# retinal-information-processing-lab/gaussian_processes

Measured on AMD Instinct MI355X. Metric: GP fits/sec (kernel+chol+solve+grad loglik) at N=8192 d=256, higher is better.
Workload: dtype f64; 1 GPU; N=8192 d=256 single cell f64, one M-step closure evaluation with 6 gradients (BASELINE configs[2], headline); N=8192, d=256, parallelism=independent units over 1 GPU(s), one process per GPU, no data-path collective

## Files before the change

gaussian_processes_amd/_lib.py:

```python
from __future__ import annotations

import ctypes
import os

from .build import lib_path

vp, i32, i64, f64 = ctypes.c_void_p, ctypes.c_int, ctypes.c_int64, ctypes.c_double
pd = ctypes.POINTER(ctypes.c_double)



class DevGemmArgs(ctypes.Structure):
    _fields_ = ([(n, vp) for n in ("A", "B", "C")] + [(n, i64) for n in ("lda", "ldb", "ldc", "sA", "sB", "sC")] +
                [("alpha", f64), ("beta", f64)] +
                [(n, vp) for n in ("sk_ws", "aux", "sumsq", "Ap", "Bp", "Cp", "auxp", "sumsqp")] +
                [(n, ctypes.c_int32) for n in ("M", "N", "K", "a_kmajor", "b_kmajor", "out_lower", "a_tri", "b_tri", "batch",
                                               "split_k", "tile", "walk", "epi", "nptr", "k_slabs")])


class DevGemmRoute(ctypes.Structure):
    _fields_ = [(n, ctypes.c_int32) for n in ("rc", "tile", "sk_first", "xcd", "stages", "half_occ", "edge", "epi",
                                              "sumsq_entries", "blocks", "pair", "slabs")]


_SIGS = {
    "gpfit_version": (i32, []),
    "gpfit_last_error": (ctypes.c_char_p, []),
    "gpfit_dgemm": (i32, [vp, i32, i32, i32, i32, i32, f64, vp, i64, vp, i64, f64, vp, i64, i32, i32, i32]),
    "gpfit_dgemm_ex": (i32, [vp, i32, i32, i32, i32, i32, f64, vp, i64, vp, i64, f64, vp, i64, i32, i32, i32, i32, i32]),
    "gpfit_ctx_create": (i32, [i32, i64, i64, i64, ctypes.POINTER(vp)]),
    "gpfit_ctx_destroy": (None, [vp]),
    "gpfit_check_limits": (i32, [pd, pd, pd]),
    "gpfit_localker_mask": (i32, [pd, i32, i32, vp, ctypes.POINTER(i64)]),
    "gpfit_localker": (i32, [vp, vp, pd, i32, i32, vp, i64, vp, vp]),
    "gpfit_acosker": (i32, [vp, vp, f64, vp, i64, i64, vp, i64, i64, i64, vp, i64, vp, vp, i64, vp]),
    "gpfit_acosker_pullback": (i32, [vp, vp, f64, vp, i64, i64, vp, i64, i64, i64, vp, i64, vp, i64, vp, vp, i64, pd]),
    "gpfit_acosker_diag": (i32, [vp, vp, f64, vp, i64, i64, i64, vp, i64, vp, vp, vp]),
    "gpfit_fit_eval": (i32, [vp, vp, pd, pd, pd, i32, i32, vp, i64, i64, vp, vp, vp, i64, f64, f64, i32, pd,
                             vp, vp, vp]),
    "gpfit_potrf": (i32, [vp, vp, vp, i64, i64, vp, i64, vp, i64, pd, ctypes.POINTER(i32)]),
    "gpfit_potrf_append": (i32, [vp, vp, vp, i64, vp, i64, i64, vp, pd, ctypes.POINTER(i32)]),
    "gpfit_potrf_append_block": (i32, [vp, vp, vp, i64, vp, i64, i64, i64, vp, i64, pd, ctypes.POINTER(i32)]),
    "gpfit_estep": (i32, [vp, vp, vp, i64, i64, vp, vp, vp, f64, vp, vp, i64]),
    "gpfit_estep_projected": (i32, [vp, vp, vp, i64, vp, i64, vp, i64, i64, i64, vp, vp, vp, f64, vp, vp, i64, vp, vp,
                                    vp]),
    "gpfit_estep_projected_damped": (i32, [vp, vp, vp, i64, vp, i64, vp, i64, vp, i64, vp, i64, i64, i64, vp, vp, vp, f64, f64,
                                           vp, vp, i64, ctypes.POINTER(i32)]),
    "gpfit_fparam_eval": (i32, [vp, vp, vp, vp, vp, i64, f64, i32, f64, vp, pd]),
    "gpfit_fparam_lbfgs": (i32, [vp, vp, vp, vp, vp, i64, f64, i32, f64, i32, i32, f64, f64, f64, vp, pd]),
    "gpfit_estep_chain": (i32, [vp, vp, vp, i64, vp, i64, vp, i64, i64, i64, vp, vp, vp, vp, vp, i64, vp, vp, f64, i32, f64,
                                i32, i32, i32, f64, f64, f64, pd]),
    "gpfit_estep_chain_full": (i32, [vp, vp, vp, i64, i64, vp, vp, vp, vp, vp, i64, vp, vp, f64, i32, f64, i32, i32, i32, f64,
                                     f64, f64, pd]),
    "gpfit_estep_chain_batch": (i32, [vp, i32, vp, vp, vp, vp, vp, vp, vp, i64, vp, vp, vp, vp, vp, vp, vp, vp, vp, pd, i32, pd,
                                      i32, i32, i32, f64, f64, f64, pd]),
# ... 8 lines not shown
    "gpfit_elbo_batch": (i32, [vp, i32, vp, vp, vp, vp, vp, vp, vp, vp, vp, ctypes.POINTER(i32), pd, vp, vp, vp, i64, pd, pd, pd,
                               ctypes.POINTER(i32)]),
    "gpfit_subspace_sweeps": (i32, [vp, vp, vp, i64, i64, i64, vp, vp, vp, vp, i32, pd, i32, ctypes.POINTER(i32)]),
    "gpfit_subspace_sweeps_batch": (i32, [vp, i32, vp, vp, i64, i64, i64, vp, vp, vp, vp, ctypes.POINTER(i32), vp, i32,
                                          ctypes.POINTER(i32)]),
    "gpfit_fparam_lbfgs_host": (i32, [vp, vp, vp, i64, f64, i32, f64, i32, i32, f64, f64, f64, vp, pd]),
    "gpfit_set_profile": (i32, [vp, i32]),
    "gpfit_get_profile": (i32, [vp, pd]),
    "gpfit_get_phases": (i32, [vp, pd]),
    "gpfit_last_enqueue_ms": (f64, [vp]),
    "gpfit_fit_eval_f32": (i32, [vp, vp, pd, pd, pd, i32, i32, vp, i64, i64, vp, vp, vp, i64, f64, f64, i32, pd,
                                 vp, vp, vp]),
    "gpfit_fit_eval_finish": (i32, [vp, pd]),
    "gpfit_fit_eval_batch": (i32, [vp, i32, vp, pd, pd, pd, i32, i32, vp, i64, i64, vp, vp, vp, i64, pd, pd, i32, pd,
                                   ctypes.POINTER(i32)]),
    "gpfit_fit_eval_batch_f32": (i32, [vp, i32, vp, pd, pd, pd, i32, i32, vp, i64, i64, vp, vp, vp, i64, pd, pd, i32, pd,
                                       ctypes.POINTER(i32)]),
    "gpfit_fit_eval_projected": (i32, [vp, vp, pd, pd, pd, i32, i32, vp, i64, i64, vp, vp, i64, i64, vp, vp, i64, f64, f64, pd]),
    "gpfit_fit_eval_projected_batch": (i32, [vp, i32, vp, pd, pd, pd, i32, i32, vp, i64, i64, vp, vp, vp, vp, vp, vp, vp, pd, pd,
                                             pd, ctypes.POINTER(i32)]),
    "gpfit_fit_eval_sparse": (i32, [vp, vp, pd, pd, pd, i32, i32, vp, i64, i64, vp, i64, i64, vp, vp, i64, i64, vp, vp, i64,
                                    f64, f64, pd]),
    "gpfit_fit_eval_sparse_batch": (i32, [vp, i32, vp, pd, pd, pd, i32, i32, vp, i64, i64, vp, i64, i64, vp, vp, vp, vp, vp,
                                          vp, vp, pd, pd, pd, ctypes.POINTER(i32)]),
    "gpfit_grad_pullback": (i32, [vp, vp, pd, i32, i32, vp, i64, i64, vp, i64, vp, pd]),
    "gpfit_nd_utility": (i32, [vp, vp, vp, i64, vp, i32, vp]),
    "gpfit_probe_mfma_f64": (i32, [vp, vp, i32, i32]),
    "gpfit_probe_stream_copy": (i32, [vp, vp, vp, i64]),
    "gpfit_dev_gemm_route": (i32, [i32, ctypes.POINTER(DevGemmArgs), ctypes.POINTER(DevGemmArgs), ctypes.POINTER(DevGemmRoute)]),
    "gpfit_dev_gemm_plan": (i64, [i32, ctypes.POINTER(DevGemmArgs), i32, ctypes.POINTER(ctypes.c_int32), i64]),
    "gpfit_dev_gemm": (i32, [vp, i32, ctypes.POINTER(DevGemmArgs), ctypes.POINTER(DevGemmArgs)]),
    "gpfit_dev_ctx_copy": (i32, [vp, ctypes.c_char_p, i64, vp, i64, i32]),
    "gpfit_dev_ctx_fill": (i32, [vp, ctypes.c_char_p, i32]),
}

_lib = None


class GpfitError(RuntimeError):
    pass


def exported_symbols():
    return sorted(_SIGS)


def load():
    global _lib
    if _lib is not None:
        return _lib
    path = lib_path()
    if not os.path.exists(path):
        raise GpfitError(
            f"{path} not found: build it with `python -m gaussian_processes_amd.build` "
            "(there is no CPU fallback for the GP fit path)")
    lib = ctypes.CDLL(path)
    for name, (res, args) in _SIGS.items():
        fn = getattr(lib, name)
        fn.restype = res
        fn.argtypes = args
    _lib = lib
    return lib


def last_error() -> str:
    return load().gpfit_last_error().decode(errors="replace")
# ... 11 lines not shown
```

gaussian_processes_amd/csrc/api_dev.hip:

```cpp
#include "gemm_core.h"
#include "context.h"
#include "gpfit_mi355x.h"

#include <cstring>

namespace gpfit {
namespace {

template <typename R>
int fill(const gpfit_dev_gemm_args& d, GemmArgsT<R>& g) {
  g = GemmArgsT<R>{};
  g.A = (const R*)d.A; g.B = (const R*)d.B; g.C = (R*)d.C;
  g.lda = d.lda; g.ldb = d.ldb; g.ldc = d.ldc;
  g.M = d.M; g.N = d.N; g.K = d.K;
  g.alpha = d.alpha; g.beta = d.beta;
  g.a_kmajor = d.a_kmajor; g.b_kmajor = d.b_kmajor;
  g.out_lower = d.out_lower; g.a_tri = d.a_tri; g.b_tri = d.b_tri;
  g.batch = d.batch > 0 ? d.batch : 1;
  g.sA = d.sA; g.sB = d.sB; g.sC = d.sC;
  g.split_k = d.split_k > 0 ? d.split_k : 1;
  g.k_slabs = d.k_slabs > 0 ? d.k_slabs : 0;
  g.tile = d.tile;
  g.reverse = d.walk & 15;
  g.half_occ = (d.walk >> 4) & 1;
  g.sk_ws = d.sk_ws;
  g.epi = d.epi;
  g.aux = (R*)d.aux;
  g.sumsq = d.sumsq;
  g.nptr = d.nptr;
  if (d.nptr < 0 || d.nptr > GEMM_MAXB) return d.nptr < 0 ? -3 : 0;
  for (int b = 0; b < d.nptr; ++b) {
    if (!d.Ap || !d.Bp || !d.Cp) return -3;
    g.Ap[b] = (const R*)d.Ap[b];
// ... 62 lines not shown
      w[3] = std::min(kr.end, (z + 1) * sp.ks * SLAB_TILE);
    }
    return need;
  }
  if (kind != 2) return -3;
  if (r.sched != GEMM_STREAMK) return -1;
  const int first = r.sk_first;
  SkHostPlan p;
  if (streamk_plan_host(a, first, p) != 0) return -1;
  const int64_t nt = (int64_t)p.tiles.size(), nfix = (int64_t)p.fix_tile.size(), nslot = (int64_t)p.fix_slot.size();
  const int64_t need = 8 + 5 * nt + nfix + (nfix + 1) + nslot;
  if (need > cap || !out) return need;
  out[0] = first; out[1] = (int32_t)nt; out[2] = p.total; out[3] = p.blocks; out[4] = p.per_block;
  out[5] = (int32_t)nfix; out[6] = (int32_t)nslot;
  out[7] = (int32_t)(SK_WS_BYTES / ((size_t)TILE * TILE * sizeof(double)));
  int32_t* w = out + 8;
  for (const SkTile& t : p.tiles) { *w++ = t.row0; *w++ = t.col0; *w++ = t.kbeg; *w++ = t.ksteps; *w++ = t.prefix; }
  std::memcpy(w, p.fix_tile.data(), nfix * sizeof(int)); w += nfix;
  std::memcpy(w, p.fix_ptr.data(), (nfix + 1) * sizeof(int)); w += nfix + 1;
  std::memcpy(w, p.fix_slot.data(), nslot * sizeof(int));
  return need;
}

template <typename R>
int run(hipStream_t s, const gpfit_dev_gemm_args& d, const gpfit_dev_gemm_args* d2) {
  GemmArgsT<R> a, b;
  if (fill(d, a) != 0 || (d2 && fill(*d2, b) != 0)) {
    set_error("gpfit_dev_gemm: a pointer batch needs its pointer arrays");
    return -3;
  }
  return d2 ? launch_gemm_pair(a, b, gemm_pair_shape(a, b), s) : launch_gemm(a, s);
}

struct CtxBuf { void* p; int64_t bytes; };
CtxBuf ctx_buffer(gpfit_ctx* c, const char* name) {
  const int64_t np = c->np_cap, dp = c->dp_cap, nn = np * np * 8;
  const struct { const char* n; double* p; int64_t bytes; } tab[] = {
      {"Abuf", c->Abuf, nn}, {"Tbuf", c->Tbuf, nn}, {"Wbuf", c->Wbuf, nn}, {"Zbuf", c->Zbuf, nn}, {"Cos", c->Cos, nn},
      {"TmpV", c->TmpV, nn}, {"Xm", c->Xm, np * dp * 8}, {"Xt2", c->Xt2, np * dp * 8}, {"Ybuf", c->Ybuf, np * dp * 8},
      {"Mmat", c->Mmat, dp * dp * 8}, {"Cmat", c->Cmat, dp * dp * 8}, {"tvec", c->tvec, 2 * np * 8}, {"bv", c->bv, np * 8},
      {"q", c->q, np * 8}, {"wl", c->wl, np * 8}, {"q2", c->q2, np * 8}, {"dq1", c->dq1, np * 8}, {"dq2", c->dq2, np * 8}};
  for (const auto& t : tab)
    if (std::strcmp(t.n, name) == 0) return {t.p, t.bytes};
  return {nullptr, 0};
}

}
}

extern "C" {

int gpfit_dev_gemm_route(int is_f32, const gpfit_dev_gemm_args* args, const gpfit_dev_gemm_args* pair_args,
                         gpfit_dev_gemm_route_t* out) {
  if (!args || !out) return -3;
  return is_f32 ? gpfit::route<float>(*args, pair_args, *out) : gpfit::route<double>(*args, pair_args, *out);
}

int64_t gpfit_dev_gemm_plan(int is_f32, const gpfit_dev_gemm_args* args, int kind, int32_t* out, int64_t cap) {
  if (!args) return -3;
  return is_f32 ? gpfit::plan<float>(*args, kind, out, cap) : gpfit::plan<double>(*args, kind, out, cap);
}

int gpfit_dev_gemm(void* stream, int is_f32, const gpfit_dev_gemm_args* args, const gpfit_dev_gemm_args* pair_args) {
  if (!args) return -3;
  return is_f32 ? gpfit::run<float>((hipStream_t)stream, *args, pair_args)
                : gpfit::run<double>((hipStream_t)stream, *args, pair_args);
}

int gpfit_dev_ctx_copy(gpfit_ctx* ctx, const char* name, int64_t offset, void* dev, int64_t bytes, int to_ctx) {
  if (!ctx || !name || !dev || offset < 0 || bytes < 0 || ctx->pend.active) return -3;
  gpfit::DeviceGuard guard(ctx->device);
  const gpfit::CtxBuf b = gpfit::ctx_buffer(ctx, name);
  if (!b.p || offset + bytes > b.bytes) return -3;
  GP_HIP(hipDeviceSynchronize());
  char* w = (char*)b.p + offset;
  GP_HIP(hipMemcpy(to_ctx ? (void*)w : dev, to_ctx ? dev : (void*)w, (size_t)bytes, hipMemcpyDeviceToDevice));
  GP_HIP(hipDeviceSynchronize());
  return 0;
}

int gpfit_dev_ctx_fill(gpfit_ctx* ctx, const char* name, int byte) {
  if (!ctx || !name || ctx->pend.active) return -3;
  gpfit::DeviceGuard guard(ctx->device);
  const gpfit::CtxBuf b = gpfit::ctx_buffer(ctx, name);
  if (!b.p) return -3;
  GP_HIP(hipDeviceSynchronize());
  GP_HIP(hipMemset(b.p, byte, (size_t)b.bytes));
  GP_HIP(hipDeviceSynchronize());
  return 0;
}

}
```

gaussian_processes_amd/csrc/common.h:

```cpp
#pragma once
#include <hip/hip_runtime.h>
#include <stdint.h>
#include <stdio.h>
#include <string>

namespace gpfit {

constexpr double PI32 = 3.1415927410125732;

constexpr int TILE = 128;
constexpr int TRMV_ROWS = 128;
constexpr int KTILE = 16;

void set_error(const std::string& msg);

#define GP_HIP(expr)                                                                     \
  do {                                                                                   \
    hipError_t _e = (expr);                                                              \
    if (_e != hipSuccess) {                                                              \
      gpfit::set_error(std::string(#expr) + ": " + hipGetErrorString(_e));               \
      return -100;                                                                       \
    }                                                                                    \
  } while (0)

#define GP_TRY(expr)            \
  do {                          \
    int _rc = (expr);           \
    if (_rc != 0) return _rc;   \
  } while (0)

inline int64_t round_up(int64_t x, int64_t m) { return (x + m - 1) / m * m; }

constexpr int GEMM_MAXB = 32;

template <typename R>
struct GemmArgsT {
  const R* A;
  const R* B;
  R* C;
  int64_t lda, ldb, ldc;
  int M, N, K;
// ... 114 lines not shown
```

gaussian_processes_amd/csrc/elementwise.hip:

```cpp
#include "kernels.h"

#include <algorithm>

namespace gpfit {

__device__ __forceinline__ double wave_sum(double v) {
#pragma unroll
  for (int o = 32; o > 0; o >>= 1) v += __shfl_down(v, o);
  return v;
}

__device__ __forceinline__ double block_sum(double v, double* sh) {
  const int lane = threadIdx.x & 63, wave = threadIdx.x >> 6;
  const int nw = (blockDim.x + 63) >> 6;
  v = wave_sum(v);
  __syncthreads();
  if (lane == 0) sh[wave] = v;
  __syncthreads();
  if (wave == 0) {
    double t = (lane < nw) ? sh[lane] : 0.0;
    t = wave_sum(t);
    if (lane == 0) sh[16] = t;
  }
  __syncthreads();
  return sh[16];
}

__device__ __forceinline__ double lin_pm1(int i, int n) {
  if (n <= 1) return -1.0;
  const double step = 2.0 / (double)(n - 1);
  return (i < n / 2) ? fma(step, (double)i, -1.0) : fma(-step, (double)(n - 1 - i), 1.0);
}

// ... 611 lines not shown
}
__global__ void dot_group_kernel(PerUnit<double*> x, PerUnit<double*> y, int n, PerUnit<double*> out) {
  __shared__ double sh[17];
  const int u = blockIdx.y;
  dot_body<double>(x[u], y[u], n, out[u], sh);
}
int launch_dot_group(int n_units, PerUnit<double*> x, PerUnit<double*> y, int n, PerUnit<double*> out, hipStream_t s) {
  hipLaunchKernelGGL(dot_group_kernel, dim3(1, n_units), dim3(1024), 0, s, x, y, n, out);
  GP_HIP(hipGetLastError());
  return 0;
}

template <typename R>
int launch_dot(const R* x, const R* y, int n, double* out, hipStream_t s) {
  hipLaunchKernelGGL(dot_kernel<R>, dim3(1), dim3(1024), 0, s, x, y, n, out);
  GP_HIP(hipGetLastError());
  return 0;
}

template <typename R>
__global__ __launch_bounds__(256) void moments_kernel(const R* __restrict__ Kvec, const R* __restrict__ q,
                                                      const R* __restrict__ Cos, int64_t ldc, const R* __restrict__ V,
                                                      int64_t ldv, const R* __restrict__ m, const R* __restrict__ r, int n,
                                                      double A, double lambda0, R* __restrict__ lam_m,
                                                      R* __restrict__ lam_var, R* __restrict__ f, R* __restrict__ wl,
                                                      double* __restrict__ scal, double* __restrict__ part,
                                                      int* __restrict__ ticket) {
  __shared__ double sh[17];
  __shared__ bool last;
  double s_rm = 0.0, s_r = 0.0, s_f = 0.0;
  const int i = blockIdx.x * 256 + threadIdx.x;
  if (i < n) {
    const double c = (double)Cos[(int64_t)i * ldc + i];
    const double delta = acos(c);
    const double J = (sqrt(1.0 - c * c) + PI32 * c - delta * c) / PI32;
    const double qi = (double)q[i];
    const double kii = qi * qi * J;
    const double lv = (double)Kvec[i] - kii + (double)V[(int64_t)i * ldv + i];
    const double lm = (double)m[i];
    const double fi = exp(A * lm + 0.5 * A * A * lv + lambda0);
    const double g = 1.0 - J - (PI32 - delta) * (1.0 - c) / PI32;
    lam_m[i] = (R)lm;
    lam_var[i] = (R)lv;
    f[i] = (R)fi;
    wl[i] = (R)(-0.5 * A * A * fi * g);
    s_rm = (double)r[i] * lm;
    s_r = (double)r[i];
    s_f = fi;
  }
  s_rm = block_sum(s_rm, sh);
  s_r = block_sum(s_r, sh);
  s_f = block_sum(s_f, sh);
  if (threadIdx.x == 0) {
    part[blockIdx.x * 3 + 0] = s_rm;
    part[blockIdx.x * 3 + 1] = s_r;
    part[blockIdx.x * 3 + 2] = s_f;
    __threadfence();
    last = (atomicAdd(ticket, 1) == (int)gridDim.x - 1);
  }
  __syncthreads();
  if (!last) return;
  __threadfence();
  if (threadIdx.x < 3) {
    double v = 0.0;
    for (int b = 0; b < (int)gridDim.x; ++b)
      v += __hip_atomic_load(&part[b * 3 + threadIdx.x], __ATOMIC_RELAXED, __HIP_MEMORY_SCOPE_AGENT);
    scal[threadIdx.x] = v;
  }
  if (threadIdx.x == 0) *ticket = 0;
}

template <typename R>
int launch_moments(const R* Kvec, const R* q, const R* Cos, int64_t ldc, const R* V, int64_t ldv, const R* m,
                   const R* r, int n, double A, double lambda0, R* lam_m, R* lam_var, R* f, R* wl, double* scal,
                   double* part, int* ticket, hipStream_t s) {
  hipLaunchKernelGGL(moments_kernel<R>, dim3((n + 255) / 256), dim3(256), 0, s, Kvec, q, Cos, ldc, V, ldv, m, r, n, A,
                     lambda0, lam_m, lam_var, f, wl, scal, part, ticket);
  GP_HIP(hipGetLastError());
  return 0;
}

template <typename R>
__global__ __launch_bounds__(256) void adjoint_kernel(const R* __restrict__ W, const R* __restrict__ Cos, int64_t ld,
                                                      const R* __restrict__ b, const R* __restrict__ q, int n,
                                                      int np, R* __restrict__ Aout, double* __restrict__ upart,
                                                      double* __restrict__ vpart, double* __restrict__ sumA_part) {
  __shared__ double colsum[4][64];
  __shared__ double sh[17];
  int ti, tj;
  {
    const int t = blockIdx.x;
    int i = (int)((sqrt(8.0 * (double)t + 1.0) - 1.0) * 0.5);
    while ((i + 1) * (i + 2) / 2 <= t) ++i;
    while (i * (i + 1) / 2 > t) --i;
    ti = i;
    tj = t - i * (i + 1) / 2;
  }
  const bool diag = (ti == tj);
  const int tx = threadIdx.x & 63, ty = threadIdx.x >> 6;
  const int j = tj * 64 + tx;
  const double qj = (double)q[j], bj = (double)b[j];
  double csum = 0.0, asum = 0.0;
  for (int rr = ty; rr < 64; rr += 4) {
    const int i = ti * 64 + rr;
    double aw = 0.0, bm = 0.0;
    if (i < n && j < n) {
      const int64_t o = (diag && i < j) ? ((int64_t)j * ld + i) : ((int64_t)i * ld + j);
      const double w = (double)W[o] - 0.5 * (double)b[i] * bj;
      const double c = (double)Cos[o];
      aw = w * (PI32 - acos(c)) / PI32;
      bm = w * sqrt(1.0 - c * c) / PI32;
    }
    Aout[(int64_t)i * ld + j] = (R)((diag && i <= j) ? (i == j ? 0.5 * aw : 0.0) : aw);
    asum += aw;
    const double rs = wave_sum(bm * qj);
    if (tx == 0) upart[(int64_t)tj * np + i] = rs;
    csum += bm * (double)q[i];
  }
  colsum[ty][tx] = csum;
  __syncthreads();
  if (!diag && ty == 0) vpart[(int64_t)ti * np + j] = colsum[0][tx] + colsum[1][tx] + colsum[2][tx] + colsum[3][tx];
  asum = block_sum(asum, sh);
  if (threadIdx.x == 0) sumA_part[blockIdx.x] = diag ? asum : 2.0 * asum;
}

template <typename R>
__global__ __launch_bounds__(256) void adjoint_u_kernel(const double* __restrict__ upart, const double* __restrict__ vpart,
                                                        int nt64, const R* __restrict__ q, const R* __restrict__ wl, int n,
                                                        int np, R* __restrict__ tvec, double* __restrict__ uq) {
  __shared__ double sl[8][33];
  const int li = threadIdx.x & 31, z = threadIdx.x >> 5;
  const int i = blockIdx.x * 32 + li;
  double u = 0.0;
  if (i < n) {
    const int T = i >> 6;
#pragma unroll 4
    for (int t = z; t < nt64; t += 8) u += (t <= T ? upart : vpart)[(int64_t)t * np + i];
  }
  sl[z][li] = u;
  __syncthreads();
  if (z != 0 || i >= np) return;
  if (i >= n) {
    tvec[i] = (R)0;
    uq[i] = 0.0;
    return;
  }
  u = sl[0][li];
#pragma unroll
  for (int k = 1; k < 8; ++k) u += sl[k][li];
  const double v = u / (double)q[i];
  uq[i] = v;
  tvec[i] = (R)(v - (double)wl[i]);
}

template <typename R>
__global__ void adjoint_sums_kernel(const double* __restrict__ uq, const R* __restrict__ wl, int n,
                                    const double* __restrict__ sumA_part, int ntile_tri, double* __restrict__ out) {
  __shared__ double sh[17];
  const int b = blockIdx.x;
  double v = 0.0;
  if (b == 0) for (int i = threadIdx.x; i < n; i += blockDim.x) v += uq[i];
  else if (b == 1) for (int i = threadIdx.x; i < n; i += blockDim.x) v += (double)wl[i];
  else for (int i = threadIdx.x; i < ntile_tri; i += blockDim.x) v += sumA_part[i];
  v = block_sum(v, sh);
  if (threadIdx.x == 0) out[b] = v;
}

__global__ __launch_bounds__(256) void adjoint_rect_kernel(const double* __restrict__ W, int64_t ldw,
                                                           const double* __restrict__ Cos, int64_t ldc,
                                                           const double* __restrict__ q1,
                                                           const double* __restrict__ q2, int n1, int n2, int np1,
                                                           int np2, double* __restrict__ Aout, int64_t lda,
                                                           double* __restrict__ upart, double* __restrict__ vpart,
                                                           double* __restrict__ tile_sum) {
  __shared__ double colsum[4][64];
  __shared__ double sh[17];
  const int tj = blockIdx.x, ti = blockIdx.y;
  const int tx = threadIdx.x & 63, ty = threadIdx.x >> 6;
  const int j = tj * 64 + tx;
  const double qj = (j < n2) ? q2[j] : 0.0;
  double csum = 0.0, asum = 0.0;
  for (int rr = ty; rr < 64; rr += 4) {
    const int i = ti * 64 + rr;
    double aw = 0.0, bm = 0.0;
    if (i < n1 && j < n2) {
      const double w = W[(int64_t)i * ldw + j];
      const double c = Cos[(int64_t)i * ldc + j];
      aw = w * (PI32 - acos(c)) / PI32;
      bm = w * sqrt(1.0 - c * c) / PI32;
    }
    Aout[(int64_t)i * lda + j] = aw;
    asum += aw;
    const double rs = wave_sum(bm * qj);
    if (tx == 0) upart[(int64_t)tj * np1 + i] = rs;
    csum += (i < n1) ? bm * q1[i] : 0.0;
  }
  colsum[ty][tx] = csum;
  __syncthreads();
  if (ty == 0) vpart[(int64_t)ti * np2 + j] = colsum[0][tx] + colsum[1][tx] + colsum[2][tx] + colsum[3][tx];
  asum = block_sum(asum, sh);
  if (threadIdx.x == 0) tile_sum[ti * gridDim.x + tj] = asum;
}

__global__ __launch_bounds__(256) void adjoint_rect_reduce_kernel(const double* __restrict__ part, int nt,
                                                                  const double* __restrict__ q,
                                                                  const double* __restrict__ extra, int n, int np,
                                                                  double* __restrict__ tvec, double* __restrict__ uq) {
  __shared__ double sl[8][33];
  const int li = threadIdx.x & 31, z = threadIdx.x >> 5;
  const int i = blockIdx.x * 32 + li;
  double u = 0.0;
  if (i < n) {
#pragma unroll 4
    for (int t = z; t < nt; t += 8) u += part[(int64_t)t * np + i];
  }
  sl[z][li] = u;
  __syncthreads();
  if (z != 0 || i >= np) return;
  if (i >= n) {
    tvec[i] = 0.0;
    uq[i] = 0.0;
    return;
  }
  u = sl[0][li];
#pragma unroll
  for (int k = 1; k < 8; ++k) u += sl[k][li];
  const double v = u / q[i];
  uq[i] = v;
// ... 168 lines not shown
  if (i >= n || j >= i) return;
  const double a = A[(int64_t)i * lda + j], b = A[(int64_t)j * lda + i];
  const double v = (a + b) / 2.0;
  A[(int64_t)i * lda + j] = v;
  A[(int64_t)j * lda + i] = v;
}
__global__ void symmetrize_avg_kernel(double* __restrict__ A, int64_t lda, int n) { symmetrize_avg_body(A, lda, n); }
__global__ void symmetrize_avg_group_kernel(PerUnit<double*> A, int64_t lda, PerUnit<int> n) {
  const int u = blockIdx.z;
  symmetrize_avg_body(A[u], lda, n[u]);
}
int launch_symmetrize_avg_group(int n_units, PerUnit<double*> A, int64_t lda, PerUnit<int> n, hipStream_t s) {
  int nmax = 0;
  for (int u = 0; u < n_units; ++u) nmax = std::max(nmax, n.v[u]);
  if (nmax <= 0) return 0;
  hipLaunchKernelGGL(symmetrize_avg_group_kernel, dim3((nmax + 255) / 256, nmax, n_units), dim3(256), 0, s, A, lda, n);
  GP_HIP(hipGetLastError());
  return 0;
}

int launch_symmetrize_avg(double* A, int64_t lda, int n, hipStream_t s) {
  hipLaunchKernelGGL(symmetrize_avg_kernel, dim3((n + 255) / 256, n), dim3(256), 0, s, A, lda, n);
  GP_HIP(hipGetLastError());
  return 0;
}

__global__ void dk_sigma0_kernel(const double* __restrict__ Cos, int64_t ldc, const double* __restrict__ q1,
                                 const double* __restrict__ q2, int n1, int n2, double s0,
                                 double* __restrict__ dK, int64_t ldk) {
  const int j = blockIdx.x * blockDim.x + threadIdx.x, i = blockIdx.y;
  if (i >= n1 || j >= n2) return;
  const double c = Cos[(int64_t)i * ldc + j];
  const double a = q1[i], b = q2[j], qq = a * b;
  const double delta = acos(c);
  const double J = (sqrt(1.0 - c * c) + PI32 * c - delta * c) / PI32;
  const double dqq = s0 * s0 * (b / a + a / b);
  const double dcos = (2.0 * s0 * s0 - c * dqq) / qq;
  const double dJ = -(delta - PI32) * dcos / PI32;
  dK[(int64_t)i * ldk + j] = (qq * dJ + dqq * J) / s0;
}

int launch_dk_sigma0(const double* Cos, int64_t ldc, const double* q1, const double* q2, int n1, int n2,
                     double s0, double* dK, int64_t ldk, hipStream_t s) {
  hipLaunchKernelGGL(dk_sigma0_kernel, dim3((n2 + 255) / 256, n1), dim3(256), 0, s, Cos, ldc, q1, q2, n1, n2, s0,
                     dK, ldk);
  GP_HIP(hipGetLastError());
  return 0;
}

__global__ void dq_kernel(const double* __restrict__ Xt, const double* __restrict__ XDt, int64_t ld, int dp,
                          int n, const double* __restrict__ q, double* __restrict__ dq, double* __restrict__ h) {
  const int i = blockIdx.x * blockDim.x + threadIdx.x;
  if (i >= n) return;
  double v = 0.0;
  for (int k = 0; k < dp; ++k) v += Xt[(int64_t)k * ld + i] * XDt[(int64_t)k * ld + i];
  if (h) h[i] = v;
  if (dq) dq[i] = 0.5 * v / q[i];
}

int launch_dq(const double* Xt, const double* XDt, int64_t ld, int dp, int n, const double* q, double* dq,
              double* h, hipStream_t s) {
  hipLaunchKernelGGL(dq_kernel, dim3((n + 255) / 256), dim3(256), 0, s, Xt, XDt, ld, dp, n, q, dq, h);
  GP_HIP(hipGetLastError());
  return 0;
}

__global__ void dk_metric_kernel(double* __restrict__ H, int64_t ldh, const double* __restrict__ Cos, int64_t ldc,
                                 const double* __restrict__ q1, const double* __restrict__ q2,
                                 const double* __restrict__ dq1, const double* __restrict__ dq2, int n1, int n2) {
  const int j = blockIdx.x * blockDim.x + threadIdx.x, i = blockIdx.y;
  if (i >= n1 || j >= n2) return;
  const double c = Cos[(int64_t)i * ldc + j];
  const double a = q1[i], b = q2[j], qq = a * b;
  const double delta = acos(c);
  const double J = (sqrt(1.0 - c * c) + PI32 * c - delta * c) / PI32;
  const double dqq = dq1[i] * b + a * dq2[j];
  const double dcos = (H[(int64_t)i * ldh + j] - c * dqq) / qq;
  const double dJ = -(delta - PI32) * dcos / PI32;
  H[(int64_t)i * ldh + j] = qq * dJ + dqq * J;
}

int launch_dk_metric(double* H, int64_t ldh, const double* Cos, int64_t ldc, const double* q1, const double* q2,
                     const double* dq1, const double* dq2, int n1, int n2, hipStream_t s) {
  hipLaunchKernelGGL(dk_metric_kernel, dim3((n2 + 255) / 256, n1), dim3(256), 0, s, H, ldh, Cos, ldc, q1, q2, dq1,
                     dq2, n1, n2);
  GP_HIP(hipGetLastError());
  return 0;
}

template <typename R>
__global__ void add_diag_kernel(R* __restrict__ A, int64_t lda, int n, double v) {
  const int i = blockIdx.x * blockDim.x + threadIdx.x;
  if (i < n) A[(int64_t)i * lda + i] += (R)v;
}

template <typename R>
int launch_add_diag(R* A, int64_t lda, int n, double v, hipStream_t s) {
  hipLaunchKernelGGL(add_diag_kernel<R>, dim3((n + 255) / 256), dim3(256), 0, s, A, lda, n, v);
  GP_HIP(hipGetLastError());
  return 0;
}
__global__ void add_diag_group_kernel(PerUnit<double*> A, int64_t lda, int n, double v) {
  const int i = blockIdx.x * blockDim.x + threadIdx.x;
  if (i < n) A[blockIdx.y][(int64_t)i * lda + i] += v;
}
int launch_add_diag_group(int n_units, PerUnit<double*> A, int64_t lda, int n, double v, hipStream_t s) {
  hipLaunchKernelGGL(add_diag_group_kernel, dim3((n + 255) / 256, n_units), dim3(256), 0, s, A, lda, n, v);
  GP_HIP(hipGetLastError());
// ... 727 lines not shown
```

gaussian_processes_amd/csrc/gram.hip:

```cpp
#include "gemm_core.h"

namespace gpfit {

template <typename R>
__global__ __launch_bounds__(GEMM_THREADS, 2) void gram_acos_kernel(GramArgsT<R> p, int tiles_n) {
  __shared__ __attribute__((aligned(16))) R smem[4 * Real<R>::KT * TILE];
  int ti, tj;
  if (p.lower) {
    tri_tile(blockIdx.x, ti, tj);
  } else {
    ti = blockIdx.x / tiles_n;
    tj = blockIdx.x % tiles_n;
  }
  const int row0 = ti * TILE, col0 = tj * TILE;
  typename Real<R>::acc_t acc[4][4];
#pragma unroll
  for (int i = 0; i < 4; ++i)
#pragma unroll
    for (int j = 0; j < 4; ++j) acc[i][j] = acc_zero<R>();

  gemm_mainloop<R, true, true, false, TILE>(p.XCt, p.ld1, p.Xt, p.ld2, p.np1, p.np2, row0, col0, 0, p.Kd, smem, acc);

  const int nv1 = p.nv1, nv2 = p.nv2;
  const bool pad_id = p.pad_identity != 0;
  const int64_t ldk = p.ldk;
  const int64_t ldcos = p.ldcos ? p.ldcos : p.ldk;
  const R s0sq = (R)p.s0sq;
  const R pi32 = (R)PI32;
  const R* __restrict__ q1 = p.q1;
  const R* __restrict__ q2 = p.q2;
  R* __restrict__ Ko = p.Kout;
  R* __restrict__ Co = p.Cos;
  const bool mirror = p.lower && p.mirror;

  for_each_acc<R, TILE>(acc, row0, col0, [&](int row, int col, R g) {
    const int64_t o = (int64_t)row * ldk + col;
    const int64_t oc = (int64_t)row * ldcos + col;
    if (mirror && row < col) return;
    if (row >= nv1 || col >= nv2) {
      if (pad_id) {
        Ko[o] = (row == col) ? (R)1 : (R)0;
        if (mirror && row > col) Ko[(int64_t)col * ldk + row] = (R)0;
        if (Co) Co[oc] = (R)0;
      }
      return;
    }
    const R qq = q1[row] * q2[col];
    R c = (g + s0sq) / (qq + (R)1e-7);
    c = fmin((R)1, fmax((R)-1, c));
    const R delta = acos(c);
    const R J = (sqrt((R)1 - c * c) + pi32 * c - delta * c) / pi32;
    Ko[o] = qq * J;
    if (mirror && row > col) Ko[(int64_t)col * ldk + row] = qq * J;
    if (Co) Co[oc] = c;
  });
}

template <typename R>
int launch_gram(const GramArgsT<R>& a, hipStream_t s) {
  if (a.nv1 <= 0 || a.nv2 <= 0) return 0;
  constexpr int EPC = 16 / (int)sizeof(R);
  if (a.Kd % ktile_of<R>() != 0 || (a.np1 % TILE) || (a.np2 % TILE) || (a.ld1 % EPC) || (a.ld2 % EPC)) {
    set_error("launch_gram: Kd must be a multiple of the K step, np1/np2 multiples of 128, ld1/ld2 of 16 bytes");
    return -3;
  }
  if (a.lower && a.np1 != a.np2) {
    set_error("launch_gram: lower needs a square problem");
    return -3;
  }
  const int tm = (a.pad_identity ? a.np1 : (int)round_up(a.nv1, TILE)) / TILE;
  const int tn = (a.pad_identity ? a.np2 : (int)round_up(a.nv2, TILE)) / TILE;
  const int tiles = a.lower ? tm * (tm + 1) / 2 : tm * tn;
  hipLaunchKernelGGL(gram_acos_kernel<R>, dim3(tiles), dim3(GEMM_THREADS), 0, s, a, tn);
  GP_HIP(hipGetLastError());
  return 0;
}

template int launch_gram<double>(const GramArgsT<double>&, hipStream_t);
template int launch_gram<float>(const GramArgsT<float>&, hipStream_t);

}
```

include/gpfit_mi355x.h:

```cpp
#ifndef GPFIT_MI355X_H
#define GPFIT_MI355X_H

#include <stdint.h>

#ifdef __cplusplus
extern "C" {
#endif

#define GPFIT_VERSION 100

int gpfit_version(void);
const char* gpfit_last_error(void);

int gpfit_dgemm(void* stream, int a_kmajor, int b_kmajor, int M, int N, int K, double alpha,
                const double* A, int64_t lda, const double* B, int64_t ldb, double beta, double* C,
                int64_t ldc, int out_lower, int a_tri, int b_tri);
int gpfit_dgemm_ex(void* stream, int a_kmajor, int b_kmajor, int M, int N, int K, double alpha,
                   const double* A, int64_t lda, const double* B, int64_t ldb, double beta, double* C,
                   int64_t ldc, int out_lower, int a_tri, int b_tri, int walk, int tile);

typedef struct gpfit_ctx gpfit_ctx;
int gpfit_ctx_create(int device, int64_t n_max, int64_t d_max, int64_t d_full_max, gpfit_ctx** out);
void gpfit_ctx_destroy(gpfit_ctx* ctx);

// ... 204 lines not shown
  int32_t M, N, K;
  int32_t a_kmajor, b_kmajor, out_lower, a_tri, b_tri;
  int32_t batch;
  int32_t split_k;
  int32_t tile;
  int32_t walk;
  int32_t epi;
  int32_t nptr;
  int32_t k_slabs;
} gpfit_dev_gemm_args;

typedef struct gpfit_dev_gemm_route_t {
  int32_t rc;
  int32_t tile;
  int32_t sk_first;
  int32_t xcd;
  int32_t stages;
  int32_t half_occ;
  int32_t edge;
  int32_t epi;
  int32_t sumsq_entries;
  int32_t blocks;
  int32_t pair;
  int32_t slabs;
} gpfit_dev_gemm_route_t;

int gpfit_dev_gemm_route(int is_f32, const gpfit_dev_gemm_args* args, const gpfit_dev_gemm_args* pair_args,
                         gpfit_dev_gemm_route_t* out);
int64_t gpfit_dev_gemm_plan(int is_f32, const gpfit_dev_gemm_args* args, int kind, int32_t* out, int64_t cap);
int gpfit_dev_gemm(void* stream, int is_f32, const gpfit_dev_gemm_args* args, const gpfit_dev_gemm_args* pair_args);
int gpfit_dev_ctx_copy(gpfit_ctx* ctx, const char* name, int64_t offset, void* dev, int64_t bytes, int to_ctx);
int gpfit_dev_ctx_fill(gpfit_ctx* ctx, const char* name, int byte);

#ifdef __cplusplus
}
#endif
#endif
```

Measured before the change: 36.64 fits/s.

## Replace library acos/sqrt with fused polynomial acos chain in gram and adjoint kernels

Adds a custom acos_chain routine that computes acos(c) and sqrt(1-c^2) together, using a shared rsq-based square root with Newton refinement and a minimax polynomial with hi/lo compensation. It is used in the gram epilogue, the diagonal, adjoint and gradient kernels in place of the separate library acos and sqrt calls, and divides by pi are replaced with multiplies by a reciprocal. The gram epilogue also gets a specialised interior path without bounds checks and with q1/q2 loads hoisted, and the adjoint kernels read b and q through wave shuffles. The transcendental cost of the epilogue is the target; accuracy now depends on the hand-written polynomial, and probe/dev entry points are added for testing.

```diff
diff --git a/gaussian_processes_amd/_lib.py b/gaussian_processes_amd/_lib.py
--- a/gaussian_processes_amd/_lib.py
+++ b/gaussian_processes_amd/_lib.py
@@ -21,6 +21,12 @@
 class DevGemmRoute(ctypes.Structure):
     _fields_ = [(n, ctypes.c_int32) for n in ("rc", "tile", "sk_first", "xcd", "stages", "half_occ", "edge", "epi",
                                               "sumsq_entries", "blocks", "pair", "slabs")]
+
+
+class DevGramArgs(ctypes.Structure):
+    _fields_ = ([(n, vp) for n in ("XCt", "Xt", "q1", "q2", "Kout", "Cos")] + [(n, i64) for n in ("ld1", "ld2", "ldk", "ldcos")] +
+                [("s0sq", f64)] +
+                [(n, ctypes.c_int32) for n in ("np1", "np2", "nv1", "nv2", "Kd", "lower", "pad_identity", "mirror")])
 
 
 _SIGS = {
@@ -95,6 +101,9 @@
     "gpfit_dev_gemm": (i32, [vp, i32, ctypes.POINTER(DevGemmArgs), ctypes.POINTER(DevGemmArgs)]),
     "gpfit_dev_ctx_copy": (i32, [vp, ctypes.c_char_p, i64, vp, i64, i32]),
     "gpfit_dev_ctx_fill": (i32, [vp, ctypes.c_char_p, i32]),
+    "gpfit_dev_acos_chain": (i32, [vp, i32, i32, vp, i64, vp, vp]),
+    "gpfit_dev_gram": (i32, [vp, i32, ctypes.POINTER(DevGramArgs)]),
+    "gpfit_dev_adjoint": (i32, [vp, i32, vp, vp, i64, vp, vp, i32, i32, vp, vp, vp, vp]),
 }
 
 _lib = None
diff --git a/gaussian_processes_amd/csrc/acos_chain.h b/gaussian_processes_amd/csrc/acos_chain.h
--- /dev/null
+++ b/gaussian_processes_amd/csrc/acos_chain.h
@@ -0,0 +1,97 @@
+#pragma once
+#include <cmath>
+
+#if defined(__HIPCC__) || defined(__CUDACC__)
+#define GPFIT_HD __host__ __device__ inline __attribute__((always_inline))
+#else
+#define GPFIT_HD inline
+#endif
+#if defined(__HIP_DEVICE_COMPILE__)
+#define GPFIT_RSQ(x, host) (sizeof(x) == 8 ? __builtin_amdgcn_rsq((double)(x)) : __builtin_amdgcn_rsqf((float)(x)))
+#else
+#define GPFIT_RSQ(x, host) ((float)(host))
+#endif
+
+namespace gpfit {
+
+#if defined(__HIP_DEVICE_COMPILE__)
+#define GPFIT_TABLE static __constant__
+#else
+#define GPFIT_TABLE static constexpr
+#endif
+GPFIT_TABLE double ACOS_H1_F64[15] = {
+    0x1.5555555555555p-1, 0x1.11111111110ddp-1, 0x1.d41d41d424b64p-2, 0x1.a01a019cbb482p-2, 0x1.7a4630d1e37b9p-2,
+    0x1.5d2cfba65c5a5p-2, 0x1.45e8811aa0db1p-2, 0x1.328ed23eb0762p-2, 0x1.24825e22e1677p-2, 0x1.0526e51d7180dp-2,
+    0x1.62bc86b4bc184p-2, -0x1.bb51923555910p-4, 0x1.3778e432526c5p+0, -0x1.71c91372389a9p+0, 0x1.b0c25ce6f2474p+0};
+GPFIT_TABLE float ACOS_H1_F32[7] = {0.6666666730944154f, 0.5333309043734016f, 0.45729240153645845f, 0.40292048509470146f,
+                                    0.4062918895403736f, 0.14373129926596173f, 0.7989290720318125f};
+
+template <typename R> struct AcosChainT;
+template <> struct AcosChainT<double> {
+  static GPFIT_HD double fma_(double a, double b, double c) { return ::fma(a, b, c); }
+  static GPFIT_HD double rsq_(double a) { return GPFIT_RSQ(a, 1.0 / ::sqrt(a)); }
+  static GPFIT_HD double abs_(double a) { return ::fabs(a); }
+  static GPFIT_HD double min_(double a, double b) { return ::fmin(a, b); }
+  static constexpr double PIO2_HI = 0x1.921fb54442d18p+0, PIO2_LO = 0x1.1a62633145c07p-54;
+  static constexpr double RSQ_MAX = 0x1p500;
+  static GPFIT_HD double h1(double z) {
+    double p = ACOS_H1_F64[14];
+#pragma unroll
+    for (int k = 13; k >= 0; --k) p = ::fma(p, z, ACOS_H1_F64[k]);
+    return p;
+  }
+};
+template <> struct AcosChainT<float> {
+  static GPFIT_HD float fma_(float a, float b, float c) { return ::fmaf(a, b, c); }
+  static GPFIT_HD float rsq_(float a) { return GPFIT_RSQ(a, 1.0f / ::sqrtf(a)); }
+  static GPFIT_HD float abs_(float a) { return ::fabsf(a); }
+  static GPFIT_HD float min_(float a, float b) { return ::fminf(a, b); }
+  static constexpr float PIO2_HI = 1.5707963705062866f, PIO2_LO = -4.371138828673793e-08f;
+  static constexpr float RSQ_MAX = 0x1p60f;
+  static GPFIT_HD float h1(float z) {
+    float p = ACOS_H1_F32[6];
+#pragma unroll
+    for (int k = 5; k >= 0; --k) p = ::fmaf(p, z, ACOS_H1_F32[k]);
+    return p;
+  }
+};
+
+template <typename R>
+GPFIT_HD R square_rounded(R a) {
+#ifdef __clang__
+#pragma clang fp contract(off)
+#endif
+  return a * a;
+}
+
+template <typename R>
+GPFIT_HD void acos_chain(R c, R& delta, R& s) {
+  using T = AcosChainT<R>;
+  const R a = T::abs_(c);
+  const bool hi = a > (R)0.5;
+  const R e = (R)1 - a;
+  const R A = hi ? e : c, B = hi ? e + e : (R)1;
+  const R w = T::fma_(-A, A, B);
+  const R wl = T::fma_(-A, A, B - w);
+  const R cc = square_rounded(c);
+  const R z = hi ? (R)0.5 * e : cc;
+  const R y = T::min_((R)T::rsq_(w), T::RSQ_MAX);
+  R g = w * y, h = (R)0.5 * y;
+  const R r = T::fma_(-h, g, (R)0.5);
+  g = T::fma_(g, r, g);
+  h = T::fma_(h, r, h);
+  g = T::fma_(T::fma_(-g, g, w), h, g);
+  g = T::fma_(T::fma_(-g, g, w), h, g);
+  const R gl = (T::fma_(-g, g, w) + wl) * h;
+  const R dw = (((R)1 - cc) - w) - wl;
+  s = g + T::fma_(dw, h, gl);
+  const R u = z * T::h1(z);
+  const bool neg = c < (R)0;
+  const R f = hi ? (neg ? (R)1 : (R)-1) : c;
+  const R kf = hi ? (neg ? (R)2 : (R)0) : (R)1;
+  const R m = f * g;
+  const R ml = T::fma_(-kf, T::PIO2_LO, T::fma_(f, gl, T::fma_(f, g, -m)));
+  delta = T::fma_(kf, T::PIO2_HI, -(m + T::fma_(m, u, ml)));
+}
+
+}
diff --git a/gaussian_processes_amd/csrc/api_dev.hip b/gaussian_processes_amd/csrc/api_dev.hip
--- a/gaussian_processes_amd/csrc/api_dev.hip
+++ b/gaussian_processes_amd/csrc/api_dev.hip
@@ -1,4 +1,6 @@
 #include "gemm_core.h"
+#include "acos_chain.h"
+#include "kernels.h"
 #include "context.h"
 #include "gpfit_mi355x.h"
 
@@ -127,6 +129,42 @@
   return d2 ? launch_gemm_pair(a, b, gemm_pair_shape(a, b), s) : launch_gemm(a, s);
 }
 
+template <typename R, bool LIBRARY>
+__global__ void acos_chain_probe_kernel(const R* __restrict__ c, int64_t n, R* __restrict__ delta, R* __restrict__ s) {
+  const int64_t i = (int64_t)blockIdx.x * blockDim.x + threadIdx.x;
+  if (i >= n) return;
+  const R ci = c[i];
+  R d, r;
+  if (LIBRARY) {
+    d = acos(ci);
+    r = sqrt((R)1 - ci * ci);
+  } else {
+    acos_chain<R>(ci, d, r);
+  }
+  delta[i] = d;
+  s[i] = r;
+}
+
+template <typename R>
+int probe_acos_chain(hipStream_t st, int library, const void* c, int64_t n, void* delta, void* s) {
+  const dim3 grid((unsigned)((n + 255) / 256)), block(256);
+  if (library) hipLaunchKernelGGL((acos_chain_probe_kernel<R, true>), grid, block, 0, st, (const R*)c, n, (R*)delta, (R*)s);
+  else hipLaunchKernelGGL((acos_chain_probe_kernel<R, false>), grid, block, 0, st, (const R*)c, n, (R*)delta, (R*)s);
+  GP_HIP(hipGetLastError());
+  return 0;
+}
+
+template <typename R>
+int run_gram(hipStream_t st, const gpfit_dev_gram_args& d) {
+  GramArgsT<R> a{};
+  a.XCt = (const R*)d.XCt; a.Xt = (const R*)d.Xt; a.q1 = (const R*)d.q1; a.q2 = (const R*)d.q2;
+  a.Kout = (R*)d.Kout; a.Cos = (R*)d.Cos;
+  a.ld1 = d.ld1; a.ld2 = d.ld2; a.ldk = d.ldk; a.ldcos = d.ldcos;
+  a.np1 = d.np1; a.np2 = d.np2; a.nv1 = d.nv1; a.nv2 = d.nv2; a.Kd = d.Kd;
+  a.s0sq = d.s0sq; a.lower = d.lower; a.pad_identity = d.pad_identity; a.mirror = d.mirror;
+  return launch_gram(a, st);
+}
+
 struct CtxBuf { void* p; int64_t bytes; };
 CtxBuf ctx_buffer(gpfit_ctx* c, const char* name) {
   const int64_t np = c->np_cap, dp = c->dp_cap, nn = np * np * 8;
@@ -162,6 +200,30 @@
                 : gpfit::run<double>((hipStream_t)stream, *args, pair_args);
 }
 
+int gpfit_dev_acos_chain(void* stream, int is_f32, int library, const void* c, int64_t n, void* delta, void* s) {
+  if (!c || !delta || !s || n < 0 || n > ((int64_t)1 << 30)) return -3;
+  if (n == 0) return 0;
+  return is_f32 ? gpfit::probe_acos_chain<float>((hipStream_t)stream, library, c, n, delta, s)
+                : gpfit::probe_acos_chain<double>((hipStream_t)stream, library, c, n, delta, s);
+}
+
+int gpfit_dev_gram(void* stream, int is_f32, const gpfit_dev_gram_args* args) {
+  if (!args || !args->XCt || !args->Xt || !args->q1 || !args->q2 || !args->Kout) return -3;
+  if (args->nv1 > args->np1 || args->nv2 > args->np2 || args->ld1 < args->np1 || args->ld2 < args->np2) return -3;
+  return is_f32 ? gpfit::run_gram<float>((hipStream_t)stream, *args) : gpfit::run_gram<double>((hipStream_t)stream, *args);
+}
+
+int gpfit_dev_adjoint(void* stream, int is_f32, const void* W, const void* Cos, int64_t ld, const void* b, const void* q,
+                      int n, int np, void* Aout, double* upart, double* vpart, double* sumA_part) {
+  if (!W || !Cos || !b || !q || !Aout || !upart || !vpart || !sumA_part) return -3;
+  if (np <= 0 || np % 64 != 0 || n <= 0 || n > np || ld < np) return -3;
+  hipStream_t st = (hipStream_t)stream;
+  return is_f32 ? gpfit::launch_adjoint<float>((const float*)W, (const float*)Cos, ld, (const float*)b, (const float*)q, n,
+                                               np, (float*)Aout, upart, vpart, sumA_part, st)
+                : gpfit::launch_adjoint<double>((const double*)W, (const double*)Cos, ld, (const double*)b,
+                                                (const double*)q, n, np, (double*)Aout, upart, vpart, sumA_part, st);
+}
+
 int gpfit_dev_ctx_copy(gpfit_ctx* ctx, const char* name, int64_t offset, void* dev, int64_t bytes, int to_ctx) {
   if (!ctx || !name || !dev || offset < 0 || bytes < 0 || ctx->pend.active) return -3;
   gpfit::DeviceGuard guard(ctx->device);
diff --git a/gaussian_processes_amd/csrc/common.h b/gaussian_processes_amd/csrc/common.h
--- a/gaussian_processes_amd/csrc/common.h
+++ b/gaussian_processes_amd/csrc/common.h
@@ -7,6 +7,7 @@
 namespace gpfit {
 
 constexpr double PI32 = 3.1415927410125732;
+constexpr double INV_PI32 = 1.0 / PI32;
 
 constexpr int TILE = 128;
 constexpr int TRMV_ROWS = 128;
diff --git a/gaussian_processes_amd/csrc/elementwise.hip b/gaussian_processes_amd/csrc/elementwise.hip
--- a/gaussian_processes_amd/csrc/elementwise.hip
+++ b/gaussian_processes_amd/csrc/elementwise.hip
@@ -1,4 +1,5 @@
 #include "kernels.h"
+#include "acos_chain.h"
 
 #include <algorithm>
 
@@ -676,8 +677,9 @@
   const int i = blockIdx.x * 256 + threadIdx.x;
   if (i < n) {
     const double c = (double)Cos[(int64_t)i * ldc + i];
-    const double delta = acos(c);
-    const double J = (sqrt(1.0 - c * c) + PI32 * c - delta * c) / PI32;
+    double delta, sn;
+    acos_chain<double>(c, delta, sn);
+    const double J = (sn + PI32 * c - delta * c) * INV_PI32;
     const double qi = (double)q[i];
     const double kii = qi * qi * J;
     const double lv = (double)Kvec[i] - kii + (double)V[(int64_t)i * ldv + i];
@@ -744,22 +746,24 @@
   const int tx = threadIdx.x & 63, ty = threadIdx.x >> 6;
   const int j = tj * 64 + tx;
   const double qj = (double)q[j], bj = (double)b[j];
+  const double brow = (double)b[ti * 64 + tx], qrow = (double)q[ti * 64 + tx];
   double csum = 0.0, asum = 0.0;
   for (int rr = ty; rr < 64; rr += 4) {
     const int i = ti * 64 + rr;
-    double aw = 0.0, bm = 0.0;
-    if (i < n && j < n) {
-      const int64_t o = (diag && i < j) ? ((int64_t)j * ld + i) : ((int64_t)i * ld + j);
-      const double w = (double)W[o] - 0.5 * (double)b[i] * bj;
-      const double c = (double)Cos[o];
-      aw = w * (PI32 - acos(c)) / PI32;
-      bm = w * sqrt(1.0 - c * c) / PI32;
-    }
+    const double bi = __shfl(brow, rr), qi = __shfl(qrow, rr);
+    const int64_t o = (diag && i < j) ? ((int64_t)j * ld + i) : ((int64_t)i * ld + j);
+    const double w = (double)W[o] - 0.5 * bi * bj;
+    const double c = (double)Cos[o];
+    double delta, sn;
+    acos_chain<double>(c, delta, sn);
+    const bool valid = i < n && j < n;
+    const double aw = valid ? w * ((PI32 - delta) * INV_PI32) : 0.0;
+    const double bm = valid ? w * (sn * INV_PI32) : 0.0;
     Aout[(int64_t)i * ld + j] = (R)((diag && i <= j) ? (i == j ? 0.5 * aw : 0.0) : aw);
     asum += aw;
     const double rs = wave_sum(bm * qj);
     if (tx == 0) upart[(int64_t)tj * np + i] = rs;
-    csum += bm * (double)q[i];
+    csum += bm * qi;
   }
   colsum[ty][tx] = csum;
   __syncthreads();
@@ -823,21 +827,25 @@
   const int tx = threadIdx.x & 63, ty = threadIdx.x >> 6;
   const int j = tj * 64 + tx;
   const double qj = (j < n2) ? q2[j] : 0.0;
+  const double qrow = (ti * 64 + tx < n1) ? q1[ti * 64 + tx] : 0.0;
   double csum = 0.0, asum = 0.0;
   for (int rr = ty; rr < 64; rr += 4) {
     const int i = ti * 64 + rr;
+    const double qi = __shfl(qrow, rr);
     double aw = 0.0, bm = 0.0;
     if (i < n1 && j < n2) {
       const double w = W[(int64_t)i * ldw + j];
       const double c = Cos[(int64_t)i * ldc + j];
-      aw = w * (PI32 - acos(c)) / PI32;
-      bm = w * sqrt(1.0 - c * c) / PI32;
+      double delta, sn;
+      acos_chain<double>(c, delta, sn);
+      aw = w * ((PI32 - delta) * INV_PI32);
+      bm = w * (sn * INV_PI32);
     }
     Aout[(int64_t)i * lda + j] = aw;
     asum += aw;
     const double rs = wave_sum(bm * qj);
     if (tx == 0) upart[(int64_t)tj * np1 + i] = rs;
-    csum += (i < n1) ? bm * q1[i] : 0.0;
+    csum += bm * qi;
   }
   colsum[ty][tx] = csum;
   __syncthreads();
@@ -1072,8 +1080,9 @@
   if (i >= n1 || j >= n2) return;
   const double c = Cos[(int64_t)i * ldc + j];
   const double a = q1[i], b = q2[j], qq = a * b;
-  const double delta = acos(c);
-  const double J = (sqrt(1.0 - c * c) + PI32 * c - delta * c) / PI32;
+  double delta, sn;
+  acos_chain<double>(c, delta, sn);
+  const double J = (sn + PI32 * c - delta * c) * INV_PI32;
   const double dqq = s0 * s0 * (b / a + a / b);
   const double dcos = (2.0 * s0 * s0 - c * dqq) / qq;
   const double dJ = -(delta - PI32) * dcos / PI32;
@@ -1112,8 +1121,9 @@
   if (i >= n1 || j >= n2) return;
   const double c = Cos[(int64_t)i * ldc + j];
   const double a = q1[i], b = q2[j], qq = a * b;
-  const double delta = acos(c);
-  const double J = (sqrt(1.0 - c * c) + PI32 * c - delta * c) / PI32;
+  double delta, sn;
+  acos_chain<double>(c, delta, sn);
+  const double J = (sn + PI32 * c - delta * c) * INV_PI32;
   const double dqq = dq1[i] * b + a * dq2[j];
   const double dcos = (H[(int64_t)i * ldh + j] - c * dqq) / qq;
   const double dJ = -(delta - PI32) * dcos / PI32;
diff --git a/gaussian_processes_amd/csrc/gram.hip b/gaussian_processes_amd/csrc/gram.hip
--- a/gaussian_processes_amd/csrc/gram.hip
+++ b/gaussian_processes_amd/csrc/gram.hip
@@ -1,6 +1,67 @@
 #include "gemm_core.h"
+#include "acos_chain.h"
 
 namespace gpfit {
+
+template <typename R, bool EDGE>
+__device__ __forceinline__ void gram_epilogue(const GramArgsT<R>& p, const typename Real<R>::acc_t (&acc)[4][4], int row0,
+                                              int col0) {
+  const int lane = threadIdx.x & 63, wave = threadIdx.x >> 6;
+  const int wm = wave >> 1, wn = wave & 1;
+  const int nv1 = p.nv1, nv2 = p.nv2;
+  const bool pad_id = p.pad_identity != 0;
+  const int64_t ldk = p.ldk;
+  const int64_t ldcos = p.ldcos ? p.ldcos : p.ldk;
+  const R s0sq = (R)p.s0sq;
+  const R pi32 = (R)PI32, inv_pi32 = (R)INV_PI32;
+  const R* __restrict__ q1 = p.q1;
+  R* __restrict__ Ko = p.Kout;
+  R* __restrict__ Co = p.Cos;
+  const bool mirror = p.lower && p.mirror;
+  const int cbase = col0 + wn * (TILE / 2) + (lane & 15);
+  R q2v[4];
+#pragma unroll
+  for (int ni = 0; ni < 4; ++ni) q2v[ni] = p.q2[cbase + ni * 16];
+#pragma unroll
+  for (int mi = 0; mi < 4; ++mi) {
+    R q1v[4];
+#pragma unroll
+    for (int r = 0; r < 4; ++r) q1v[r] = q1[row0 + wm * (TILE / 2) + mi * 16 + Real<R>::crow(lane, r)];
+#pragma unroll
+    for (int r = 0; r < 4; ++r) {
+      const int row = row0 + wm * (TILE / 2) + mi * 16 + Real<R>::crow(lane, r);
+      R* __restrict__ Krow = Ko + (int64_t)row * ldk;
+      R* __restrict__ Crow = Co ? Co + (int64_t)row * ldcos : nullptr;
+#pragma unroll
+      for (int ni = 0; ni < 4; ++ni) {
+        const int col = cbase + ni * 16;
+        const R qq = q1v[r] * q2v[ni];
+        R c = (acc[mi][ni][r] + s0sq) / (qq + (R)1e-7);
+        c = fmin((R)1, fmax((R)-1, c));
+        R delta, sn;
+        acos_chain<R>(c, delta, sn);
+        const R J = (sn + pi32 * c - delta * c) * inv_pi32;
+        const R k = qq * J;
+        if (!EDGE) {
+          Krow[col] = k;
+          if (mirror) Ko[(int64_t)col * ldk + row] = k;
+          if (Crow) Crow[col] = c;
+        } else {
+          if (mirror && row < col) continue;
+          if (row < nv1 && col < nv2) {
+            Krow[col] = k;
+            if (mirror && row > col) Ko[(int64_t)col * ldk + row] = k;
+            if (Crow) Crow[col] = c;
+          } else if (pad_id) {
+            Krow[col] = (row == col) ? (R)1 : (R)0;
+            if (mirror && row > col) Ko[(int64_t)col * ldk + row] = (R)0;
+            if (Crow) Crow[col] = (R)0;
+          }
+        }
+      }
+    }
+  }
+}
 
 template <typename R>
 __global__ __launch_bounds__(GEMM_THREADS, 2) void gram_acos_kernel(GramArgsT<R> p, int tiles_n) {
@@ -21,39 +82,9 @@
 
   gemm_mainloop<R, true, true, false, TILE>(p.XCt, p.ld1, p.Xt, p.ld2, p.np1, p.np2, row0, col0, 0, p.Kd, smem, acc);
 
-  const int nv1 = p.nv1, nv2 = p.nv2;
-  const bool pad_id = p.pad_identity != 0;
-  const int64_t ldk = p.ldk;
-  const int64_t ldcos = p.ldcos ? p.ldcos : p.ldk;
-  const R s0sq = (R)p.s0sq;
-  const R pi32 = (R)PI32;
-  const R* __restrict__ q1 = p.q1;
-  const R* __restrict__ q2 = p.q2;
-  R* __restrict__ Ko = p.Kout;
-  R* __restrict__ Co = p.Cos;
-  const bool mirror = p.lower && p.mirror;
-
-  for_each_acc<R, TILE>(acc, row0, col0, [&](int row, int col, R g) {
-    const int64_t o = (int64_t)row * ldk + col;
-    const int64_t oc = (int64_t)row * ldcos + col;
-    if (mirror && row < col) return;
-    if (row >= nv1 || col >= nv2) {
-      if (pad_id) {
-        Ko[o] = (row == col) ? (R)1 : (R)0;
-        if (mirror && row > col) Ko[(int64_t)col * ldk + row] = (R)0;
-        if (Co) Co[oc] = (R)0;
-      }
-      return;
-    }
-    const R qq = q1[row] * q2[col];
-    R c = (g + s0sq) / (qq + (R)1e-7);
-    c = fmin((R)1, fmax((R)-1, c));
-    const R delta = acos(c);
-    const R J = (sqrt((R)1 - c * c) + pi32 * c - delta * c) / pi32;
-    Ko[o] = qq * J;
-    if (mirror && row > col) Ko[(int64_t)col * ldk + row] = qq * J;
-    if (Co) Co[oc] = c;
-  });
+  const bool inside = row0 + TILE <= p.nv1 && col0 + TILE <= p.nv2 && !(p.lower && p.mirror && ti == tj);
+  if (inside) gram_epilogue<R, false>(p, acc, row0, col0);
+  else gram_epilogue<R, true>(p, acc, row0, col0);
 }
 
 template <typename R>
diff --git a/include/gpfit_mi355x.h b/include/gpfit_mi355x.h
--- a/include/gpfit_mi355x.h
+++ b/include/gpfit_mi355x.h
@@ -260,6 +260,22 @@
 int gpfit_dev_ctx_copy(gpfit_ctx* ctx, const char* name, int64_t offset, void* dev, int64_t bytes, int to_ctx);
 int gpfit_dev_ctx_fill(gpfit_ctx* ctx, const char* name, int byte);
 
+int gpfit_dev_acos_chain(void* stream, int is_f32, int library, const void* c, int64_t n, void* delta, void* s);
+typedef struct gpfit_dev_gram_args {
+  const void* XCt;
+  const void* Xt;
+  const void* q1;
+  const void* q2;
+  void* Kout;
+  void* Cos;
+  int64_t ld1, ld2, ldk, ldcos;
+  double s0sq;
+  int32_t np1, np2, nv1, nv2, Kd, lower, pad_identity, mirror;
+} gpfit_dev_gram_args;
+int gpfit_dev_gram(void* stream, int is_f32, const gpfit_dev_gram_args* args);
+int gpfit_dev_adjoint(void* stream, int is_f32, const void* W, const void* Cos, int64_t ld, const void* b, const void* q,
+                      int n, int np, void* Aout, double* upart, double* vpart, double* sumA_part);
+
 #ifdef __cplusplus
 }
 #endif
```

New measurement: 36.89 fits/s (median of 6 runs). About the same (+0.7%).
